# lxtGH/Video-K-Net

Hardware: AMD Instinct MI355X
Metric: frames/sec (S=3, N=100, 1024x2048) (higher is better)
Workload: dtype f32; 1 GPU; cfg2 video_knet_s3_r50: VideoKernelIterHead S=3, N=100 proposals + 17 stuff = 117 kernels, C=256, 1024x2048 frame -> 128x256 stride-8 features, ffn tracking link, x4 bilinear upsample of the final logits; streams_per_gpu=1, parallelism=frame-sharded dp1, x_storage=fp32

## Files before the change

include/vkn.h:

```cpp
#ifndef VKN_H
#define VKN_H
#include <stddef.h>
#include <stdint.h>

#ifdef __cplusplus
extern "C" {
#endif

#define VKN_VERSION 0x000600

#define VKN_OK 0
#define VKN_E_ARG (-1)
#define VKN_E_SHAPE (-2)
#define VKN_E_WORKSPACE (-3)
#define VKN_E_LAUNCH (-4)
#define VKN_E_ALIGN (-5)
#define VKN_E_RANGE (-6)

#define VKN_STATUS_RANGE 1u

#define VKN_FLAG_REF_KERNELS 1u
#define VKN_FLAG_EXACT_GEMM 2u
#define VKN_FLAG_LOGITS_HANDOFF 4u
#define VKN_FLAG_BITS_HANDOFF 16u
#define VKN_X_F32 0
#define VKN_X_F16 1
#define VKN_X_BF16 2
#define VKN_FLAG_X_F16 64u
#define VKN_FLAG_X_BF16 128u
#define VKN_FLAG_CHAIN_LAUNCHES 256u
#define VKN_FLAG_CHAIN_PERSISTENT 512u
#define VKN_FLAG_JOIN_EARLY 32768u
#define VKN_FLAG_LINK_RESERVE 262144u
#define VKN_FLAG_LINK_NO_RESERVE 524288u
#define VKN_FLAG_SCALED_F16 16384u
#define VKN_FLAG_CHAIN_BF16X3 65536u
#define VKN_FLAG_CHAIN_KSPLIT 8192u
#define VKN_FLAG_SERIAL_LINK 32u
#define VKN_FLAG_CLIP_LINK 8u

#define VKN_FLAG_INIT_SEPARATE 131072u
#define VKN_FLAG_PHASE_A 1024u
#define VKN_FLAG_PHASE_B 2048u
#define VKN_FLAG_PHASE_C 4096u
#define VKN_FLAG_PHASE_MASK (VKN_FLAG_PHASE_A | VKN_FLAG_PHASE_B | VKN_FLAG_PHASE_C)

#define VKN_MAX_FCS 4

typedef struct VknDims {
    int B;
    int N;
    int C;
    int H, W;
    int heads;
    int ff;
    int ncls;
    int n_cls_fcs, n_mask_fcs;
    float thr_logit;
    float ln_eps;
} VknDims;

typedef struct VknStageWeights {
    const float *ft_w, *ft_b, *ft_wT;
    const float *dyn_w, *dyn_b;
    const float *inp_w, *inp_b;
    const float *ig_w, *ig_b, *ug_w, *ug_b;
    const float *norm_in_w, *norm_in_b;
    const float *norm_out_w, *norm_out_b;
    const float *inorm_in_w, *inorm_in_b;
// ... 346 lines not shown
```

video-k-net_amd/csrc/vkn_api.hip:

```cpp
#include "../../include/vkn.h"
#include "../../include/vkn_decode.h"
#include "vkn_common.h"
#include "vkn_launch.h"

namespace {

struct Carver {
    char* base;
    size_t off;
    template <class T>
    T* take(size_t n) {
        off = (off + 255) & ~(size_t)255;
        T* p = base ? reinterpret_cast<T*>(base + off) : nullptr;
        off += n * sizeof(T);
        return p;
    }
};

inline bool aligned16(const void* p) { return (reinterpret_cast<uintptr_t>(p) & 15) == 0; }
inline int npt_of(int N) { return (N + 31) / 32 * 32; }

struct StageWs {
    float *part, *cntp, *xraw, *cnt, *xfeat, *params, *inputf, *ig, *ug, *f, *obj1, *qkv, *ao, *obj2, *h, *partial, *t1, *t2,
        *maskfeat, *kb, *kern32, *lq, *lkv, *lobj, *lupd, *lf;
// ... 401 lines not shown
        const long long q = grid * 3 / 4;
        return (int)(q > full ? full : (q < d->B ? d->B : q));
    }
    if (mode != 1 || !persistent_chain || d->B < VKN_LINK_RESERVE_MIN_FRAMES || xdt_of(flags) != 0) return 0;
    return grid == VKN_DECODE_CUS ? full : 0;
}

inline int persistent_min_row_tiles(const PrepW& pw, unsigned flags) {
    return (!(flags & VKN_FLAG_CHAIN_BF16X3) && pw.h2_scale && pw.h2[VKN_H2_DYNFT]) ? 22 : 64;
}
inline unsigned pw_off(const VknStageWeights* w, const void* p) {
    return (unsigned)(static_cast<const char*>(p) - static_cast<const char*>(w->prepared));
}
inline bool chain_weights_ok(const PrepW& pw, bool have_cls) {
    return pw.dynft && pw.dyn && pw.dec && pw.inp && pw.ig && pw.ug && pw.fc && pw.attn_in && pw.attn_out && pw.ffn1 && pw.ffn2 &&
           pw.cls_fc[0] && pw.mask_fc[0] && (!have_cls || pw.fc_cls);
}
inline bool chain_stage_ok(const VknDims* d, const VknStageWeights* w, const PrepW& pw, bool have_cls) {
    return chain_shape_ok(d) && w->prepared && w->prepared_bytes < (1ull << 31) && chain_weights_ok(pw, have_cls) && w->ffn1_w &&
           w->cls_ln_w[0] && w->mask_ln_w[0];
}
bool chain_fast_ok(const VknDims* d, const VknStageWeights* w, const PrepW& pw, unsigned flags, bool have_cls) {
    if (flags & (VKN_FLAG_CHAIN_LAUNCHES | VKN_FLAG_EXACT_GEMM)) return false;
    if (vkn_dbg_env("VKN_CHAIN_LAUNCHES", 0)) return false;
    if (!(flags & VKN_FLAG_CHAIN_PERSISTENT) && !vkn_dbg_env("VKN_CHAIN_PERSISTENT", 0) &&
        (d->B * d->N + 31) / 32 < persistent_min_row_tiles(pw, flags))
        return false;
    return pw.chain_consts && chain_stage_ok(d, w, pw, have_cls);
}
inline bool chain_h2(const PrepW& pw, unsigned flags, bool have_cls) {
    return !(flags & VKN_FLAG_CHAIN_BF16X3) && pw.h2_scale && pw.h2[VKN_H2_DYNFT] && pw.h2[VKN_H2_DEC] && (!have_cls || pw.h2[VKN_H2_FCCLS]);
}

int run_chain_fast(const VknDims* d, const VknStageWeights* w, const PrepW& pw, const float* a0, bool a0_raw, const float* cnt,
                   const float* obj_in, float* obj_out, float* cls_logits, bool cls_sigmoid, float* kern32_out, const StageWs& s,
                   hipStream_t st, bool h2 = false) {
    const int M = d->B * d->N, C = d->C;
    VknChainA a{};
    a.a0 = a0; a.obj_in = obj_in; a.rowscale = a0_raw ? cnt : nullptr;
    a.wbase = w->prepared; a.wbytes = w->prepared_bytes;
    if (h2) {
        a.off_dyn = pw_off(w, pw.h2[a0_raw ? VKN_H2_DYNFT : VKN_H2_DYN]);
        a.off_inp = pw_off(w, pw.h2[VKN_H2_INP]); a.off_ig = pw_off(w, pw.h2[VKN_H2_IG]); a.off_ug = pw_off(w, pw.h2[VKN_H2_UG]);
        a.off_fc = pw_off(w, pw.h2[VKN_H2_FC]); a.off_in = pw_off(w, pw.h2[VKN_H2_IN]);
    } else {
        a.off_dyn = pw_off(w, a0_raw ? pw.dynft : pw.dyn);
        a.off_inp = pw_off(w, pw.inp); a.off_ig = pw_off(w, pw.ig); a.off_ug = pw_off(w, pw.ug); a.off_fc = pw_off(w, pw.fc);
        a.off_in = pw_off(w, pw.attn_in);
    }
    a.consts = pw.chain_consts;
    a.eps = d->ln_eps; a.M = M; a.obj1 = s.obj1; a.qkv = s.qkv; a.status = s.status;
    VKN_TRY(h2 ? vkn_launch_chain_a_h2(a, st) : vkn_launch_chain_a(a, st));
    VKN_TRY(vkn_launch_attn(s.qkv, 3 * C, s.qkv + C, s.qkv + 2 * C, 3 * C, s.ao, C, d->B, d->N, d->N, d->heads, C / d->heads, st));
    VknChainC c{};
    c.ao = s.ao; c.obj1 = s.obj1; c.wbase = w->prepared; c.wbytes = w->prepared_bytes;
    if (h2) {
        c.off_out = pw_off(w, pw.h2[VKN_H2_OUT]); c.off_ffn1 = pw_off(w, pw.h2[VKN_H2_FFN1]); c.off_ffn2 = pw_off(w, pw.h2[VKN_H2_FFN2]);
        c.off_clsfc = pw_off(w, pw.h2[VKN_H2_CLSFC]); c.off_maskfc = pw_off(w, pw.h2[VKN_H2_MASKFC]);
        c.off_fccls = pw.h2[VKN_H2_FCCLS] ? pw_off(w, pw.h2[VKN_H2_FCCLS]) : 0u; c.off_dec = pw_off(w, pw.h2[VKN_H2_DEC]);
    } else {
        c.off_out = pw_off(w, pw.attn_out); c.off_ffn1 = pw_off(w, pw.ffn1); c.off_ffn2 = pw_off(w, pw.ffn2);
        c.off_clsfc = pw_off(w, pw.cls_fc[0]); c.off_maskfc = pw_off(w, pw.mask_fc[0]);
        c.off_fccls = pw.fc_cls ? pw_off(w, pw.fc_cls) : 0u; c.off_dec = pw_off(w, pw.dec);
    }
    c.consts = pw.chain_consts; c.kb0 = pw.kb0;
    c.ff = d->ff; c.ncls = d->ncls; c.cls_sigmoid = cls_sigmoid ? 1 : 0; c.eps = d->ln_eps; c.M = M;
    c.obj_out = obj_out; c.cls_out = cls_logits; c.kb_out = s.kb;
    if (kern32_out) c.kern_out = kern32_out;
    else { c.plane_hi = s.kfh; c.plane_lo = s.kfl; }
    c.rows_per_frame = d->N; c.NPT = npt_of(d->N); c.status = s.status;
    return h2 ? vkn_launch_chain_c_h2(c, st) : vkn_launch_chain_c(c, st);
}

#define VKN_KS_MAX_ROW_TILES 16
inline bool ks_width_ok(const VknDims* d) {
    return chain_width_ok(d) && (d->ff % 512 == 0 || d->ff <= 1024);
}
bool chain_ks_ok(const VknDims* d, const VknStageWeights* w, const PrepW& pw, unsigned flags, bool have_cls) {
    if (flags & (VKN_FLAG_CHAIN_LAUNCHES | VKN_FLAG_CHAIN_PERSISTENT | VKN_FLAG_EXACT_GEMM)) return false;
    if (vkn_dbg_env("VKN_CHAIN_LAUNCHES", 0) || vkn_dbg_env("VKN_CHAIN_PERSISTENT", 0) || !vkn_dbg_env("VKN_CHAIN_KSPLIT", 1)) return false;
    if (!(flags & VKN_FLAG_CHAIN_KSPLIT) && (d->B * d->N + 31) / 32 > VKN_KS_MAX_ROW_TILES) return false;
    if (!ks_width_ok(d) || !chain_stage_ok(d, w, pw, have_cls)) return false;
    const void* v16[] = {w->inorm_in_w, w->inorm_in_b, w->norm_in_w, w->norm_in_b, w->norm_out_w, w->norm_out_b, w->inorm_out_w, w->inorm_out_b,
                         w->fc_norm_w, w->fc_norm_b, w->attn_norm_w, w->attn_norm_b, w->ffn_norm_w, w->ffn_norm_b, w->ffn2_b,
                         w->cls_ln_w[0], w->cls_ln_b[0], w->mask_ln_w[0], w->mask_ln_b[0], pw.dvec};
    for (const void* p : v16)
        if (!p || !aligned16(p)) return false;
    return true;
}

VknKsProb ks_prob(const float* a, int lda, const void* W, int Nout, int KT, float eps) {
    VknKsProb p{};
    p.pro.a[0] = a; p.pro.lda[0] = lda; p.pro.nsum = 1; p.pro.eps = eps;
    p.Wsplit = W; p.Nout = Nout; p.KT = KT;
    return p;
}

int run_chain_ks(const VknDims* d, const VknStageWeights* w, const PrepW& pw, const float* a0, bool a0_raw, const float* cnt,
                 const float* obj_in, float* obj_out, float* cls_logits, bool cls_sigmoid, float* kern32_out, const StageWs& s,
                 hipStream_t st, hipEvent_t obj_ready) {
    const int M = d->B * d->N, C = d->C, FF = d->ff;
    const float eps = d->ln_eps;
    VknKsProb pr[2];
// ... 147 lines not shown
                           will_fast ? w->prepared_bytes : 0));

    float* xfeat = c.x_feat_out ? c.x_feat_out : s.xfeat;
    VknEpi e = mk_epi(d);
    if (given_xfeat) {
        xfeat = const_cast<float*>(c.xfeat_in);
    } else if (has_ft) {
        if (!comp || c.x_feat_out || need_xfeat) {
            e.bias = w->ft_b; e.rowscale = s.cnt; e.out = xfeat; e.ldo = C;
            VKN_TRY(vkn_launch_gemm(s.xraw, nullptr, C, w->ft_w, pw.ft, M, C, C, 1, nullptr, e, st));
        }
    } else {
        if (hipMemcpyAsync(xfeat, s.xraw, (size_t)M * C * sizeof(float), hipMemcpyDeviceToDevice, st) != hipSuccess)
            return VKN_E_LAUNCH;
    }

    const float* obj_in = c.obj_in;
    if (pre_link) {
        PrepW pl;
        VKN_TRY(carve_pw(d, c.link_pre, flags, &pl));
        VKN_TRY(run_link(d, c.link_pre, pl, obj_in, c.prev_pre, s.lobj, s, st, c.link_pre->dyn_w ? xfeat : nullptr, flags));
        obj_in = s.lobj;
    }

    const float* kb = has_ft ? s.kb : nullptr;
    float* const kern32 = ref_decode ? (chain_only ? c.kern_out : s.kern32) : nullptr;
    const bool link = c.prev_obj && c.track_out;
    if (fast) {
        const bool raw = !given_xfeat;
        if (fewrow) {
            VKN_TRY(run_chain_ks(d, w, pw, raw ? s.xraw : xfeat, raw, s.cnt, obj_in, c.obj_out, cls_logits, c.cls_sigmoid, kern32, s, st, c.obj_ready));
        } else {
            VKN_TRY(run_chain_fast(d, w, pw, raw ? s.xraw : xfeat, raw, s.cnt, obj_in, c.obj_out, cls_logits, c.cls_sigmoid, kern32, s, st,
                                   chain_h2(pw, flags, have_cls)));
            if (c.obj_ready && hipEventRecord(c.obj_ready, st) != hipSuccess) return VKN_E_LAUNCH;
        }
        VKN_TRY(emit_masks(d, c, s, ref_decode, s.kern32, kb, touch_nx, touch_nx_bytes, flags, st, !fewrow));
        if (link) VKN_TRY(run_track_link(d, s, st, c.obj_out, c.prev_obj, c.track_out, w, c.link_track, c.track_src, xfeat, flags));
        return VKN_OK;
    }

    VKN_TRY(run_updator(d, w, pw, xfeat, (comp && !given_xfeat) ? s.xraw : nullptr, s.cnt, obj_in, s.obj1, s, st));

    VKN_TRY(run_attention(d, s, s.obj1, s.obj1, d->heads, w->attn_in_w, pw.attn_in, nullptr, w->attn_in_b, w->attn_out_w,
                          pw.attn_out, w->attn_out_b, w->attn_norm_w, w->attn_norm_b, s.obj2, st));
    if (w->ffn1_w) {
        VKN_TRY(run_ffn(d, s, s.obj2, w->ffn1_w, pw.ffn1, w->ffn1_b, w->ffn2_w, pw.ffn2, w->ffn2_b, w->ffn_norm_w,
                        w->ffn_norm_b, c.obj_out, st));
    } else {
        if (hipMemcpyAsync(c.obj_out, s.obj2, (size_t)M * C * sizeof(float), hipMemcpyDeviceToDevice, st) != hipSuccess)
            return VKN_E_LAUNCH;
    }
    const float* obj3 = c.obj_out;

    const bool fork_late = vkn_dbg_env("VKN_LINK_FORK_LATE", 0) != 0;
    if (c.obj_ready && !fork_late && hipEventRecord(c.obj_ready, st) != hipSuccess) return VKN_E_LAUNCH;

    const float* tc = obj3;
    const float* tm = obj3;
    const int nl = d->n_cls_fcs > d->n_mask_fcs ? d->n_cls_fcs : d->n_mask_fcs;
    VknGemmProb pr[2];
    for (int i = 0; i < nl; ++i) {
        int np = 0;
        if (i < d->n_cls_fcs) {
            float* dst = (i & 1) ? s.t2 : s.t1;
            e = mk_epi(d); e.ln_w = w->cls_ln_w[i]; e.ln_b = w->cls_ln_b[i]; e.act = 1; e.out = dst; e.ldo = C;
            pr[np++] = VknGemmProb{tc, nullptr, nullptr, nullptr, C, w->cls_fc_w[i], pw.cls_fc[i], C, e};
// ... 871 lines not shown
```

video-k-net_amd/csrc/vkn_chain.hip:

```cpp
#include "vkn_common.h"
#include "vkn_launch.h"

#ifdef CH_H2
typedef _Float16 ch_e;
#define CH_NPL 2
#define CH_WTILE 32768u
#define k_chain_a k_chain_a_h2
#define k_chain_c k_chain_c_h2
#define ChainAArgs ChainAArgsH2
#define ChainCArgs ChainCArgsH2
#define vkn_launch_chain_a vkn_launch_chain_a_h2
#define vkn_launch_chain_c vkn_launch_chain_c_h2
#else
typedef __bf16 ch_e;
#define CH_NPL 3
#define CH_WTILE 49152u
#endif
typedef ch_e ch_ex8 __attribute__((ext_vector_type(8)));
typedef ch_e ch_ex4 __attribute__((ext_vector_type(4)));
typedef unsigned int cu32x4 __attribute__((ext_vector_type(4)));

#define CH_THREADS 512
#define CH_ROWS 32
#define CH_C 256
#define CH_IMG (CH_NPL * CH_ROWS * CH_C)
#define CH_PLANE (CH_ROWS * CH_C)
#define CH_SBUF (2 * 16 * 32)

#define CH_BAR() asm volatile("s_waitcnt lgkmcnt(0)\n\ts_barrier" ::: "memory")

namespace {

__device__ __forceinline__ void ch_split(float v, ch_e (&p)[CH_NPL]) {
    float r = v;
#pragma unroll
    for (int i = 0; i < CH_NPL; ++i) {
        p[i] = (ch_e)r;
        if (i + 1 < CH_NPL) r -= (float)p[i];
    }
}
__device__ __forceinline__ void ch_split4(const float (&v)[4], ch_ex4 (&o)[CH_NPL]) {
// ... 530 lines not shown
    CC_B2 = 768, CC_FN_W = 1024, CC_FN_B = 1280,
    CC_CLN_W = 1536, CC_CLN_B = 1792,
    CC_MLN_W = 2048, CC_MLN_B = 2304,
    CC_DVEC = 2560,
    CC_CLS_B = 2816,
    CC_DEC_B = 3072,
    CC_B1 = 3328,
    CC_SC = 3328 + 2048,
    CC_TOTAL = 3328 + 2048 + 8
};

struct ChainCArgs {
    const float* ao;
    const float* obj1;
    const void* wbase;
    unsigned wbytes;
    unsigned off_out, off_ffn1, off_ffn2, off_clsfc, off_maskfc, off_fccls, off_dec;
    int nchunks;
    int has_cls;
    int cls_sigmoid;
    int ncls;
    float eps;
    int M;
    const float* kb0;
    float* obj_out;
    float* cls_out;
    float* kb_out;
    _Float16* plane_hi;
    _Float16* plane_lo;
    float* kern_out;
    int rows_per_frame, NPT;
    const float* consts;
    int* status;
};

template <int ABL>
__global__ __launch_bounds__(CH_THREADS) void k_chain_c(const ChainCArgs A) {
    extern __shared__ __attribute__((aligned(16))) char smem_cc[];
    ch_e* IMG0 = reinterpret_cast<ch_e*>(smem_cc);
    ch_e* HID = IMG0 + CH_IMG;
    float* S = reinterpret_cast<float*>(HID + CH_IMG);
    float* CST = S + 2 * CH_SBUF;
#ifdef CH_H2
    float* RS = CST + CC_TOTAL;
#endif

    const int tid = threadIdx.x;
    ChLane L_ = ch_lane(tid);
    L_.status = A.status;
    const ChLane L = L_;
    const int m0 = blockIdx.x * CH_ROWS, M = A.M;
    const int row = m0 + L.li;
    const bool row_ok = row < M;
    const int rowc = min(row, M - 1);
    const __amdgpu_buffer_rsrc_t wrs = __builtin_amdgcn_make_buffer_rsrc(const_cast<void*>(A.wbase), 0, (int)A.wbytes, 0x00020000);

    constexpr int RING = CH_RING_OF(ABL);
    ChRing<RING> R;
    {
        const ChNext first{A.off_out, 0u, 1};
#pragma unroll
        for (int j = 0; j < RING - 1; ++j) ch_wload<RING, CH_AUX_OF(ABL), CH_NP_OF(ABL)>(R, j, wrs, L, first.off(j));
        if (CH_NOLOAD(ABL)) ch_wload<RING>(R, RING - 1, wrs, L, A.off_out);
    }
    ch_stage_consts<CC_TOTAL>(CST, A.consts, tid);
#ifdef CH_H2
    ch_img_load(IMG0, A.ao, CH_C, m0, M, tid, RS);
#else
    ch_img_load(IMG0, A.ao, CH_C, m0, M, tid);
#endif
    float obj[1][16];
    {
        const float* s = A.obj1 + (size_t)rowc * CH_C + L.wave * 32 + 4 * L.g;
#pragma unroll
        for (int q = 0; q < 4; ++q) {
            const f32x4 t = *reinterpret_cast<const f32x4*>(s + 8 * q);
#pragma unroll
            for (int e = 0; e < 4; ++e) obj[0][4 * q + e] = t[e];
        }
    }
    CH_BAR();

    int sb = 0;
    f32x16 acc1[1];
    ch_zero(acc1[0]);
    ch_gemm<1, true, ABL>(acc1, IMG0, IMG0, A.off_out, 0u, ChNext{A.off_ffn1, 0u, 1}, R, wrs, L);
    CH_UNSCALE(acc1[0], CST[CC_SC + 0] * RS[L.li]);
    {
        float b[16];
        ch_cols(CST + CC_OUT_B, L, b);
#pragma unroll
        for (int r = 0; r < 16; ++r) obj[0][r] = acc1[0][r] + b[r] + obj[0][r];
        const float* const lw[1] = {CST + CC_AN_W};
        const float* const lb[1] = {CST + CC_AN_B};
        ch_layernorm<1>(obj, lw, lb, A.eps, S, sb, L);
        ch_img_write(IMG0, obj[0], L);
        CH_BAR();
    }
    f32x16 acc2[1];
    ch_zero(acc2[0]);
#pragma unroll 1
    for (int c = 0; c < A.nchunks; ++c) {
        ch_zero(acc1[0]);
        ch_gemm<1, true, ABL>(acc1, IMG0, IMG0, A.off_ffn1 + (unsigned)c * 8u * CH_WTILE, 0u,
                         ChNext{A.off_ffn2 + (unsigned)c * 8u * CH_WTILE, 0u, 1}, R, wrs, L);
        CH_UNSCALE(acc1[0], CST[CC_SC + 1]);
        float h[16], b[16];
        ch_cols(CST + CC_B1 + 256 * c, L, b);
#pragma unroll
        for (int r = 0; r < 16; ++r) h[r] = fmaxf(acc1[0][r] + b[r], 0.f);
        CH_BAR();
        ch_img_write(HID, h, L);
        CH_BAR();
        const bool lastc = (c + 1 == A.nchunks);
        const ChNext nx = lastc ? ChNext{A.off_clsfc, A.off_maskfc, 2} : ChNext{A.off_ffn1 + (unsigned)(c + 1) * 8u * CH_WTILE, 0u, 1};
        ch_gemm<1, true, ABL>(acc2, HID, HID, A.off_ffn2 + (unsigned)c * 8u * CH_WTILE, 0u, nx, R, wrs, L);
    }
    CH_UNSCALE(acc2[0], CST[CC_SC + 2]);
    {
        float b[16];
        ch_cols(CST + CC_B2, L, b);
#pragma unroll
        for (int r = 0; r < 16; ++r) obj[0][r] = obj[0][r] + acc2[0][r] + b[r];
        const float* const lw[1] = {CST + CC_FN_W};
        const float* const lb[1] = {CST + CC_FN_B};
        ch_layernorm<1>(obj, lw, lb, A.eps, S, sb, L);
        ch_store_rows(A.obj_out, CH_C, 0, row, row_ok, obj[0], L);
        ch_img_write(IMG0, obj[0], L);
        CH_BAR();
    }
    f32x16 acc[2];
    ch_zero(acc[0]);
    ch_zero(acc[1]);
    const ChNext nfin = A.has_cls ? ChNext{A.off_fccls, A.off_dec, 2} : ChNext{A.off_dec, 0u, 1};
    ch_gemm<2, true, ABL>(acc, IMG0, IMG0, A.off_clsfc, A.off_maskfc, nfin, R, wrs, L);
    CH_UNSCALE(acc[0], CST[CC_SC + 3]);
    CH_UNSCALE(acc[1], CST[CC_SC + 4]);
    {
        float t[2][16];
#pragma unroll
        for (int r = 0; r < 16; ++r) {
            t[0][r] = acc[0][r];
            t[1][r] = acc[1][r];
        }
        const float* const lw[2] = {CST + CC_CLN_W, CST + CC_MLN_W};
        const float* const lb[2] = {CST + CC_CLN_B, CST + CC_MLN_B};
        ch_layernorm<2>(t, lw, lb, A.eps, S, sb, L);
        float dv[16], kd[1];
        ch_cols(CST + CC_DVEC, L, dv);
// ... 29 lines not shown
    } else {
        f32x16 accd[1];
        ch_zero(accd[0]);
        ch_gemm<1, true, ABL>(accd, HID, HID, A.off_dec, 0u, ChNext{0u, 0u, 0}, R, wrs, L);
        acc[1] = accd[0];
    }
    CH_UNSCALE(acc[1], CST[CC_SC + 6]);
    {
        float k[16], b[16];
        ch_cols(CST + CC_DEC_B, L, b);
#pragma unroll
        for (int r = 0; r < 16; ++r) k[r] = acc[1][r] + b[r];
        if (A.plane_hi) {
            if (row_ok) {
                const int fb = row / A.rows_per_frame, n = row - fb * A.rows_per_frame;
                const size_t base = ((size_t)fb * A.NPT + n) * CH_C + L.wave * 32 + 4 * L.g;
#pragma unroll
                for (int q = 0; q < 4; ++q) {
                    half4 h, l;
#pragma unroll
                    for (int e = 0; e < 4; ++e) {
                        _Float16 hh, ll;
                        vkn_split_f16(k[4 * q + e], hh, ll);
                        h[e] = hh;
                        l[e] = ll;
                    }
                    *reinterpret_cast<half4*>(A.plane_hi + base + 8 * q) = h;
                    *reinterpret_cast<half4*>(A.plane_lo + base + 8 * q) = l;
                }
            }
        } else {
            ch_store_rows(A.kern_out, CH_C, 0, row, row_ok, k, L);
        }
    }
}

#ifndef CH_H2
template <int ABL, int KC>
__global__ __launch_bounds__(CH_THREADS) void k_gemm_t3(const VknGemmProb p0, const VknGemmProb p1, int nprob, int M) {
    extern __shared__ __attribute__((aligned(16))) char smem_t3[];
    ch_e* IMG = reinterpret_cast<ch_e*>(smem_t3);
    float* S = reinterpret_cast<float*>(IMG + KC * CH_IMG);
    const bool second = (nprob > 1) && (blockIdx.z == 1);
    const VknGemmProb& P = second ? p1 : p0;
    const VknEpi& E = P.epi;
    const int Nout = P.Nout;
    const int m0 = blockIdx.y * CH_ROWS, n0 = blockIdx.x * 256;
    if (n0 >= Nout) return;

    const int tid = threadIdx.x;
    const ChLane L = ch_lane(tid);
    const int ntiles = (Nout + 255) / 256;
    const __amdgpu_buffer_rsrc_t wrs = __builtin_amdgcn_make_buffer_rsrc(const_cast<void*>(P.Wsplit), 0, (int)((unsigned)ntiles * (8u * KC) * CH_WTILE), 0x00020000);
    const unsigned wbase = (unsigned)blockIdx.x * (8u * KC) * CH_WTILE;
    constexpr int RING = CH_RING_OF(ABL);
    ChRing<RING> R;
#pragma unroll
    for (int j = 0; j < RING - 1; ++j) ch_wload<RING, CH_AUX_OF(ABL)>(R, j, wrs, L, wbase + (unsigned)j * CH_WTILE);

#pragma unroll
    for (int kc = 0; kc < KC; ++kc) {
        const int row = tid >> 4, c4 = (tid & 15) << 2;
        const size_t ro = (size_t)min(m0 + row, M - 1) * P.lda + c4 + 256 * kc;
        f32x4 t[4];
#pragma unroll
        for (int j = 0; j < 4; ++j) t[j] = *reinterpret_cast<const f32x4*>(P.A + ro + 64 * j);
// ... 294 lines not shown
        case 2: CHA_LAUNCH(2); break;
        case 3: CHA_LAUNCH(3); break;
        case 4: CHA_LAUNCH(4); break;
        case 5: CHA_LAUNCH(5); break;
        case 6: CHA_LAUNCH(6); break;
        case 7: CHA_LAUNCH(7); break;
        case 8: CHA_LAUNCH(8); break;
        case 9: CHA_LAUNCH(9); break;
        case 10: CHA_LAUNCH(10); break;
        case 11: CHA_LAUNCH(11); break;
        default: CHA_LAUNCH(0); break;
    }
#else
    CHA_LAUNCH(0);
#endif
#undef CHA_LAUNCH
    VKN_CHECK_LAUNCH();
    return VKN_OK;
}

int vkn_launch_chain_c(const VknChainC& p, hipStream_t stream) {
    if (!p.ao || !p.obj1 || !p.wbase || !p.obj_out || !p.consts || p.M <= 0 || p.wbytes >= (1ull << 31)) return VKN_E_ARG;
    if (p.ff <= 0 || p.ff % 256 != 0 || p.ff > 2048 || p.ncls > 256) return VKN_E_SHAPE;
    if (!p.plane_hi == !p.kern_out || (p.plane_hi && !p.plane_lo)) return VKN_E_ARG;
    ChainCArgs A{};
    A.ao = p.ao; A.obj1 = p.obj1; A.wbase = p.wbase; A.wbytes = (unsigned)p.wbytes;
    A.off_out = p.off_out; A.off_ffn1 = p.off_ffn1; A.off_ffn2 = p.off_ffn2; A.off_clsfc = p.off_clsfc; A.off_maskfc = p.off_maskfc;
    A.off_fccls = p.off_fccls; A.off_dec = p.off_dec;
    A.nchunks = p.ff / 256; A.has_cls = (p.cls_out != nullptr) ? 1 : 0; A.cls_sigmoid = p.cls_sigmoid; A.ncls = p.ncls;
    A.eps = p.eps; A.M = p.M; A.kb0 = p.kb0; A.obj_out = p.obj_out; A.cls_out = p.cls_out; A.kb_out = p.kb_out;
    A.plane_hi = p.plane_hi; A.plane_lo = p.plane_lo; A.kern_out = p.kern_out; A.rows_per_frame = p.rows_per_frame; A.NPT = p.NPT;
    A.consts = p.consts + 2 * CA_TOTAL;
    A.status = p.status;
#ifdef CH_H2
    const size_t lds = (size_t)2 * CH_IMG * sizeof(ch_e) + (size_t)(2 * CH_SBUF + CC_TOTAL + 32) * sizeof(float);
#else
    const size_t lds = (size_t)2 * CH_IMG * sizeof(ch_e) + (size_t)(2 * CH_SBUF + CC_TOTAL) * sizeof(float);
#endif
#define CHC_LAUNCH(ABLV)                                                                                            \
    do {                                                                                                            \
        VKN_ALLOW_FULL_LDS(k_chain_c<ABLV>);                                                                        \
        hipLaunchKernelGGL(k_chain_c<ABLV>, dim3((p.M + CH_ROWS - 1) / CH_ROWS), dim3(CH_THREADS), lds, stream, A); \
    } while (0)
#ifdef VKN_DEBUG
    switch (vkn_dbg_env("VKN_CHAIN_ABL", 0)) {
        case 1: CHC_LAUNCH(1); break;
        case 2: CHC_LAUNCH(2); break;
        case 3: CHC_LAUNCH(3); break;
        case 4: CHC_LAUNCH(4); break;
        case 5: CHC_LAUNCH(5); break;
        case 6: CHC_LAUNCH(6); break;
        case 7: CHC_LAUNCH(7); break;
        case 8: CHC_LAUNCH(8); break;
        case 9: CHC_LAUNCH(9); break;
        case 10: CHC_LAUNCH(10); break;
        case 11: CHC_LAUNCH(11); break;
        default: CHC_LAUNCH(0); break;
    }
#else
    CHC_LAUNCH(0);
#endif
#undef CHC_LAUNCH
    VKN_CHECK_LAUNCH();
    return VKN_OK;
}
```

video-k-net_amd/csrc/vkn_launch.h:

```cpp
#pragma once
#include <hip/hip_runtime.h>
#include <stddef.h>

struct VknEpi {
    const float* bias;
    const float* rowscale;
    const float* bias2;
    const float* resid;
    int ldr;
    const float* ln_w;
    const float* ln_b;
    int ln_from_col;
    float eps;
    int act;
    float* out;
    int ldo;
    const float* dot_vec;
    const float* dot_bias;
    float* dot_out;
    _Float16* plane_hi;
    _Float16* plane_lo;
    int rows_per_frame;
    int NPT;
};
// ... 112 lines not shown
int vkn_chain_pack_consts(const VknChainConsts& c, float* out, hipStream_t stream);
struct VknChainA {
    const float* a0;
    const float* obj_in;
    const float* rowscale;
    const void* wbase;
    size_t wbytes;
    unsigned off_dyn, off_inp, off_ig, off_ug, off_fc, off_in;
    const float* consts;
    float eps;
    int M;
    float* obj1;
    float* qkv;
    int* status;
};
struct VknChainC {
    const float* ao;
    const float* obj1;
    const void* wbase;
    size_t wbytes;
    unsigned off_out, off_ffn1, off_ffn2, off_clsfc, off_maskfc, off_fccls, off_dec;
    const float* consts;
    const float* kb0;
    int ff, ncls, cls_sigmoid;
    float eps;
    int M;
    float* obj_out;
    float* cls_out;
    float* kb_out;
    _Float16 *plane_hi, *plane_lo;
    float* kern_out;
    int rows_per_frame, NPT;
    int* status;
};
int vkn_launch_gemm_t3(const VknGemmProb* probs, int nprob, int M, int K, hipStream_t stream);
int vkn_launch_chain_a(const VknChainA& p, hipStream_t stream);
int vkn_launch_chain_c(const VknChainC& p, hipStream_t stream);
int vkn_launch_chain_a_h2(const VknChainA& p, hipStream_t stream);
int vkn_launch_chain_c_h2(const VknChainC& p, hipStream_t stream);
size_t vkn_split_h2_bytes(int Nout, int K);
int vkn_launch_split_h2(const float* W, void* images, int Nout, int K, const float* scale, hipStream_t stream);

struct VknKsPro {
    const float* a[4];
    int lda[4];
    int nsum;
    long long sum_stride;
    const float* pbias;
    const float* presid;
    int ldr;
    const float* ln_w[4];
    const float* ln_b[4];
    float eps;
    int act;
    float* side_out;
    int ld_side;
    const float* dot_vec;
    const float* dot_bias;
    float* dot_out;
};
struct VknKsEpi {
    const float* bias;
    const float* rowscale;
    const float* bias2;
    const float* resid;
    int ldr;
// ... 17 lines not shown
```

video-k-net_amd/ops.py:

```python
import ctypes
import struct
import threading

import torch

from . import _lib
from ._lib import VknDims, VknStageWeights, check

_H = _lib.CONSTS
FLAG_REF_KERNELS = _H['VKN_FLAG_REF_KERNELS']
FLAG_EXACT_GEMM = _H['VKN_FLAG_EXACT_GEMM']
FLAG_LOGITS_HANDOFF = _H['VKN_FLAG_LOGITS_HANDOFF']
FLAG_BITS_HANDOFF = _H['VKN_FLAG_BITS_HANDOFF']
FLAG_CHAIN_LAUNCHES = _H['VKN_FLAG_CHAIN_LAUNCHES']
FLAG_CHAIN_PERSISTENT = _H['VKN_FLAG_CHAIN_PERSISTENT']
FLAG_JOIN_EARLY = _H['VKN_FLAG_JOIN_EARLY']
FLAG_LINK_RESERVE = _H['VKN_FLAG_LINK_RESERVE']
FLAG_LINK_NO_RESERVE = _H['VKN_FLAG_LINK_NO_RESERVE']
FLAG_SCALED_F16 = _H['VKN_FLAG_SCALED_F16']
FLAG_CHAIN_BF16X3 = _H['VKN_FLAG_CHAIN_BF16X3']
FLAG_INIT_SEPARATE = _H['VKN_FLAG_INIT_SEPARATE']
FLAG_CHAIN_KSPLIT = _H['VKN_FLAG_CHAIN_KSPLIT']
FLAG_SERIAL_LINK = _H['VKN_FLAG_SERIAL_LINK']

_tls = threading.local()


def _ptr(t):
    return ctypes.c_void_p(t.data_ptr()) if t is not None else ctypes.c_void_p(0)


def _stream():
    return ctypes.c_void_p(torch.cuda.current_stream().cuda_stream)


def _req(t, name):
    if not torch.is_tensor(t) or not t.is_cuda:
        raise _lib.VknLibraryError(f'{name}: expected a CUDA/HIP tensor — the MI355X path has no CPU fallback')
    if t.dtype != torch.float32:
        raise TypeError(f'{name}: expected float32, got {t.dtype}')
    t = t.contiguous()
    if t.data_ptr() % 16:
        t = t.clone(memory_format=torch.contiguous_format)
    return t


_X_DTYPES = {torch.float32: _H['VKN_X_F32'], torch.float16: _H['VKN_X_F16'], torch.bfloat16: _H['VKN_X_BF16']}
FLAG_X_F16, FLAG_X_BF16 = _H['VKN_FLAG_X_F16'], _H['VKN_FLAG_X_BF16']


def _req_x(t, name='x'):
    if not torch.is_tensor(t) or not t.is_cuda:
        raise _lib.VknLibraryError(f'{name}: expected a CUDA/HIP tensor — the MI355X path has no CPU fallback')
# ... 1259 lines not shown
```

Measured before the change: 9915 frames/s.

## Split chain C kernel across FFN hidden chunks into partial and reduce kernels

```diff
diff --git a/include/vkn.h b/include/vkn.h
--- a/include/vkn.h
+++ b/include/vkn.h
@@ -35,6 +35,7 @@
 #define VKN_FLAG_LINK_NO_RESERVE 524288u
 #define VKN_FLAG_SCALED_F16 16384u
 #define VKN_FLAG_CHAIN_BF16X3 65536u
+#define VKN_FLAG_CHAIN_WHOLE_C 1048576u
 #define VKN_FLAG_CHAIN_KSPLIT 8192u
 #define VKN_FLAG_SERIAL_LINK 32u
 #define VKN_FLAG_CLIP_LINK 8u
diff --git a/video-k-net_amd/csrc/vkn_api.hip b/video-k-net_amd/csrc/vkn_api.hip
--- a/video-k-net_amd/csrc/vkn_api.hip
+++ b/video-k-net_amd/csrc/vkn_api.hip
@@ -457,9 +457,17 @@
     return !(flags & VKN_FLAG_CHAIN_BF16X3) && pw.h2_scale && pw.h2[VKN_H2_DYNFT] && pw.h2[VKN_H2_DEC] && (!have_cls || pw.h2[VKN_H2_FCCLS]);
 }
 
+int chain_c_hsplit(int M, int FF, unsigned flags) {
+    if (flags & VKN_FLAG_CHAIN_WHOLE_C) return 1;
+    const int chunks = FF / 256, rt = (M + 31) / 32;
+    int hs = 1;
+    while (chunks % (hs * 2) == 0 && rt * hs * 2 <= VKN_DECODE_CUS) hs *= 2;
+    return hs;
+}
+
 int run_chain_fast(const VknDims* d, const VknStageWeights* w, const PrepW& pw, const float* a0, bool a0_raw, const float* cnt,
                    const float* obj_in, float* obj_out, float* cls_logits, bool cls_sigmoid, float* kern32_out, const StageWs& s,
-                   hipStream_t st, bool h2 = false) {
+                   hipStream_t st, bool h2 = false, int c_hsplit = 1) {
     const int M = d->B * d->N, C = d->C;
     VknChainA a{};
     a.a0 = a0; a.obj_in = obj_in; a.rowscale = a0_raw ? cnt : nullptr;
@@ -494,6 +502,7 @@
     if (kern32_out) c.kern_out = kern32_out;
     else { c.plane_hi = s.kfh; c.plane_lo = s.kfl; }
     c.rows_per_frame = d->N; c.NPT = npt_of(d->N); c.status = s.status;
+    c.hsplit = c_hsplit; c.obj2 = s.obj2; c.partial = s.partial;
     return h2 ? vkn_launch_chain_c_h2(c, st) : vkn_launch_chain_c(c, st);
 }
 
@@ -707,7 +716,7 @@
             VKN_TRY(run_chain_ks(d, w, pw, raw ? s.xraw : xfeat, raw, s.cnt, obj_in, c.obj_out, cls_logits, c.cls_sigmoid, kern32, s, st, c.obj_ready));
         } else {
             VKN_TRY(run_chain_fast(d, w, pw, raw ? s.xraw : xfeat, raw, s.cnt, obj_in, c.obj_out, cls_logits, c.cls_sigmoid, kern32, s, st,
-                                   chain_h2(pw, flags, have_cls)));
+                                   chain_h2(pw, flags, have_cls), chain_c_hsplit(M, d->ff, flags)));
             if (c.obj_ready && hipEventRecord(c.obj_ready, st) != hipSuccess) return VKN_E_LAUNCH;
         }
         VKN_TRY(emit_masks(d, c, s, ref_decode, s.kern32, kb, touch_nx, touch_nx_bytes, flags, st, !fewrow));
diff --git a/video-k-net_amd/csrc/vkn_chain.hip b/video-k-net_amd/csrc/vkn_chain.hip
--- a/video-k-net_amd/csrc/vkn_chain.hip
+++ b/video-k-net_amd/csrc/vkn_chain.hip
@@ -7,6 +7,8 @@
 #define CH_WTILE 32768u
 #define k_chain_a k_chain_a_h2
 #define k_chain_c k_chain_c_h2
+#define k_chain_c1 k_chain_c1_h2
+#define k_chain_c2 k_chain_c2_h2
 #define ChainAArgs ChainAArgsH2
 #define ChainCArgs ChainCArgsH2
 #define vkn_launch_chain_a vkn_launch_chain_a_h2
@@ -603,7 +605,71 @@
     int rows_per_frame, NPT;
     const float* consts;
     int* status;
+    float* obj2;
+    float* part;
+    int hs;
 };
+
+template <int ABL>
+__device__ __forceinline__ void ch_c_front(const ChainCArgs& A, ch_e* IMG0, float* S, float* CST, float* RS, int& sb, float (&obj)[1][16],
+                                           ChRing<CH_RING_OF(ABL)>& R, const __amdgpu_buffer_rsrc_t wrs, const ChLane& L, int tid, int m0,
+                                           int rowc, const ChNext nx) {
+    constexpr int RING = CH_RING_OF(ABL);
+    {
+        const ChNext first{A.off_out, 0u, 1};
+#pragma unroll
+        for (int j = 0; j < RING - 1; ++j) ch_wload<RING, CH_AUX_OF(ABL), CH_NP_OF(ABL)>(R, j, wrs, L, first.off(j));
+        if (CH_NOLOAD(ABL)) ch_wload<RING>(R, RING - 1, wrs, L, A.off_out);
+    }
+    ch_stage_consts<CC_TOTAL>(CST, A.consts, tid);
+#ifdef CH_H2
+    ch_img_load(IMG0, A.ao, CH_C, m0, A.M, tid, RS);
+#else
+    ch_img_load(IMG0, A.ao, CH_C, m0, A.M, tid);
+#endif
+    {
+        const float* s = A.obj1 + (size_t)rowc * CH_C + L.wave * 32 + 4 * L.g;
+#pragma unroll
+        for (int q = 0; q < 4; ++q) {
+            const f32x4 t = *reinterpret_cast<const f32x4*>(s + 8 * q);
+#pragma unroll
+            for (int e = 0; e < 4; ++e) obj[0][4 * q + e] = t[e];
+        }
+    }
+    CH_BAR();
+
+    f32x16 acc1[1];
+    ch_zero(acc1[0]);
+    ch_gemm<1, true, ABL>(acc1, IMG0, IMG0, A.off_out, 0u, nx, R, wrs, L);
+    CH_UNSCALE(acc1[0], CST[CC_SC + 0] * RS[L.li]);
+    float b[16];
+    ch_cols(CST + CC_OUT_B, L, b);
+#pragma unroll
+    for (int r = 0; r < 16; ++r) obj[0][r] = acc1[0][r] + b[r] + obj[0][r];
+    const float* const lw[1] = {CST + CC_AN_W};
+    const float* const lb[1] = {CST + CC_AN_B};
+    ch_layernorm<1>(obj, lw, lb, A.eps, S, sb, L);
+    ch_img_write(IMG0, obj[0], L);
+    CH_BAR();
+}
+
+template <int ABL>
+__device__ __forceinline__ void ch_ffn_chunk(const ChainCArgs& A, int c, f32x16 (&acc2)[1], const ch_e* IMG0, ch_e* HID, const float* CST,
+                                             ChRing<CH_RING_OF(ABL)>& R, const __amdgpu_buffer_rsrc_t wrs, const ChLane& L, const ChNext nx) {
+    f32x16 acc1[1];
+    ch_zero(acc1[0]);
+    ch_gemm<1, true, ABL>(acc1, IMG0, IMG0, A.off_ffn1 + (unsigned)c * 8u * CH_WTILE, 0u,
+                     ChNext{A.off_ffn2 + (unsigned)c * 8u * CH_WTILE, 0u, 1}, R, wrs, L);
+    CH_UNSCALE(acc1[0], CST[CC_SC + 1]);
+    float h[16], b[16];
+    ch_cols(CST + CC_B1 + 256 * c, L, b);
+#pragma unroll
+    for (int r = 0; r < 16; ++r) h[r] = fmaxf(acc1[0][r] + b[r], 0.f);
+    CH_BAR();
+    ch_img_write(HID, h, L);
+    CH_BAR();
+    ch_gemm<1, true, ABL>(acc2, HID, HID, A.off_ffn2 + (unsigned)c * 8u * CH_WTILE, 0u, nx, R, wrs, L);
+}
 
 template <int ABL>
 __global__ __launch_bounds__(CH_THREADS) void k_chain_c(const ChainCArgs A) {
@@ -614,6 +680,8 @@
     float* CST = S + 2 * CH_SBUF;
 #ifdef CH_H2
     float* RS = CST + CC_TOTAL;
+#else
+    float* RS = nullptr;
 #endif
 
     const int tid = threadIdx.x;
@@ -626,66 +694,17 @@
     const int rowc = min(row, M - 1);
     const __amdgpu_buffer_rsrc_t wrs = __builtin_amdgcn_make_buffer_rsrc(const_cast<void*>(A.wbase), 0, (int)A.wbytes, 0x00020000);
 
-    constexpr int RING = CH_RING_OF(ABL);
-    ChRing<RING> R;
-    {
-        const ChNext first{A.off_out, 0u, 1};
-#pragma unroll
-        for (int j = 0; j < RING - 1; ++j) ch_wload<RING, CH_AUX_OF(ABL), CH_NP_OF(ABL)>(R, j, wrs, L, first.off(j));
-        if (CH_NOLOAD(ABL)) ch_wload<RING>(R, RING - 1, wrs, L, A.off_out);
-    }
-    ch_stage_consts<CC_TOTAL>(CST, A.consts, tid);
-#ifdef CH_H2
-    ch_img_load(IMG0, A.ao, CH_C, m0, M, tid, RS);
-#else
-    ch_img_load(IMG0, A.ao, CH_C, m0, M, tid);
-#endif
+    ChRing<CH_RING_OF(ABL)> R;
+    int sb = 0;
     float obj[1][16];
-    {
-        const float* s = A.obj1 + (size_t)rowc * CH_C + L.wave * 32 + 4 * L.g;
-#pragma unroll
-        for (int q = 0; q < 4; ++q) {
-            const f32x4 t = *reinterpret_cast<const f32x4*>(s + 8 * q);
-#pragma unroll
-            for (int e = 0; e < 4; ++e) obj[0][4 * q + e] = t[e];
-        }
-    }
-    CH_BAR();
-
-    int sb = 0;
-    f32x16 acc1[1];
-    ch_zero(acc1[0]);
-    ch_gemm<1, true, ABL>(acc1, IMG0, IMG0, A.off_out, 0u, ChNext{A.off_ffn1, 0u, 1}, R, wrs, L);
-    CH_UNSCALE(acc1[0], CST[CC_SC + 0] * RS[L.li]);
-    {
-        float b[16];
-        ch_cols(CST + CC_OUT_B, L, b);
-#pragma unroll
-        for (int r = 0; r < 16; ++r) obj[0][r] = acc1[0][r] + b[r] + obj[0][r];
-        const float* const lw[1] = {CST + CC_AN_W};
-        const float* const lb[1] = {CST + CC_AN_B};
-        ch_layernorm<1>(obj, lw, lb, A.eps, S, sb, L);
-        ch_img_write(IMG0, obj[0], L);
-        CH_BAR();
-    }
+    ch_c_front<ABL>(A, IMG0, S, CST, RS, sb, obj, R, wrs, L, tid, m0, rowc, ChNext{A.off_ffn1, 0u, 1});
     f32x16 acc2[1];
     ch_zero(acc2[0]);
 #pragma unroll 1
     for (int c = 0; c < A.nchunks; ++c) {
-        ch_zero(acc1[0]);
-        ch_gemm<1, true, ABL>(acc1, IMG0, IMG0, A.off_ffn1 + (unsigned)c * 8u * CH_WTILE, 0u,
-                         ChNext{A.off_ffn2 + (unsigned)c * 8u * CH_WTILE, 0u, 1}, R, wrs, L);
-        CH_UNSCALE(acc1[0], CST[CC_SC + 1]);
-        float h[16], b[16];
-        ch_cols(CST + CC_B1 + 256 * c, L, b);
-#pragma unroll
-        for (int r = 0; r < 16; ++r) h[r] = fmaxf(acc1[0][r] + b[r], 0.f);
-        CH_BAR();
-        ch_img_write(HID, h, L);
-        CH_BAR();
         const bool lastc = (c + 1 == A.nchunks);
         const ChNext nx = lastc ? ChNext{A.off_clsfc, A.off_maskfc, 2} : ChNext{A.off_ffn1 + (unsigned)(c + 1) * 8u * CH_WTILE, 0u, 1};
-        ch_gemm<1, true, ABL>(acc2, HID, HID, A.off_ffn2 + (unsigned)c * 8u * CH_WTILE, 0u, nx, R, wrs, L);
+        ch_ffn_chunk<ABL>(A, c, acc2, IMG0, HID, CST, R, wrs, L, nx);
     }
     CH_UNSCALE(acc2[0], CST[CC_SC + 2]);
     {
@@ -781,6 +800,195 @@
         } else {
             ch_store_rows(A.kern_out, CH_C, 0, row, row_ok, k, L);
         }
+    }
+}
+
+template <int ABL>
+__global__ __launch_bounds__(CH_THREADS) void k_chain_c1(const ChainCArgs A) {
+    extern __shared__ __attribute__((aligned(16))) char smem_c1[];
+    ch_e* IMG0 = reinterpret_cast<ch_e*>(smem_c1);
+    ch_e* HID = IMG0 + CH_IMG;
+    float* S = reinterpret_cast<float*>(HID + CH_IMG);
+    float* CST = S + 2 * CH_SBUF;
+#ifdef CH_H2
+    float* RS = CST + CC_TOTAL;
+#else
+    float* RS = nullptr;
+#endif
+
+    const int tid = threadIdx.x;
+    ChLane L_ = ch_lane(tid);
+    L_.status = A.status;
+    const ChLane L = L_;
+    const int m0 = blockIdx.x * CH_ROWS, M = A.M;
+    const int row = m0 + L.li;
+    const bool row_ok = row < M;
+    const int rowc = min(row, M - 1);
+    const int grp = blockIdx.y, cpg = A.nchunks / A.hs, cbeg = grp * cpg, cend = cbeg + cpg;
+    const __amdgpu_buffer_rsrc_t wrs = __builtin_amdgcn_make_buffer_rsrc(const_cast<void*>(A.wbase), 0, (int)A.wbytes, 0x00020000);
+
+    ChRing<CH_RING_OF(ABL)> R;
+    int sb = 0;
+    float obj[1][16];
+    ch_c_front<ABL>(A, IMG0, S, CST, RS, sb, obj, R, wrs, L, tid, m0, rowc, ChNext{A.off_ffn1 + (unsigned)cbeg * 8u * CH_WTILE, 0u, 1});
+    if (grp == 0) ch_store_rows(A.obj2, CH_C, 0, row, row_ok, obj[0], L);
+    f32x16 acc2[1];
+    ch_zero(acc2[0]);
+#pragma unroll 1
+    for (int c = cbeg; c < cend; ++c) {
+        const ChNext nx = (c + 1 == cend) ? ChNext{0u, 0u, 0} : ChNext{A.off_ffn1 + (unsigned)(c + 1) * 8u * CH_WTILE, 0u, 1};
+        ch_ffn_chunk<ABL>(A, c, acc2, IMG0, HID, CST, R, wrs, L, nx);
+    }
+    CH_UNSCALE(acc2[0], CST[CC_SC + 2]);
+    {
+        float v[16];
+#pragma unroll
+        for (int r = 0; r < 16; ++r) v[r] = acc2[0][r];
+        ch_store_rows(A.part + (size_t)grp * M * CH_C, CH_C, 0, row, row_ok, v, L);
+    }
+}
+
+template <int ABL>
+__global__ __launch_bounds__(CH_THREADS) void k_chain_c2(const ChainCArgs A) {
+    extern __shared__ __attribute__((aligned(16))) char smem_c2[];
+    ch_e* IMG0 = reinterpret_cast<ch_e*>(smem_c2);
+    float* S = reinterpret_cast<float*>(IMG0 + CH_IMG);
+    float* CST = S + 2 * CH_SBUF;
+
+    const int tid = threadIdx.x;
+    ChLane L_ = ch_lane(tid);
+    L_.status = A.status;
+    const ChLane L = L_;
+    const int m0 = blockIdx.x * CH_ROWS, M = A.M;
+    const int row = m0 + L.li;
+    const bool row_ok = row < M;
+    const int rowc = min(row, M - 1);
+    const bool is_cls = A.has_cls && blockIdx.y == 0;
+    const unsigned off_fc = is_cls ? A.off_clsfc : A.off_maskfc, off_fin = is_cls ? A.off_fccls : A.off_dec;
+    const __amdgpu_buffer_rsrc_t wrs = __builtin_amdgcn_make_buffer_rsrc(const_cast<void*>(A.wbase), 0, (int)A.wbytes, 0x00020000);
+
+    constexpr int RING = CH_RING_OF(ABL);
+    ChRing<RING> R;
+    {
+        const ChNext first{off_fc, 0u, 1};
+#pragma unroll
+        for (int j = 0; j < RING - 1; ++j) ch_wload<RING, CH_AUX_OF(ABL), CH_NP_OF(ABL)>(R, j, wrs, L, first.off(j));
+        if (CH_NOLOAD(ABL)) ch_wload<RING>(R, RING - 1, wrs, L, off_fc);
+    }
+    ch_stage_consts<CC_TOTAL>(CST, A.consts, tid);
+    float obj[1][16];
+    {
+        const size_t ro = (size_t)rowc * CH_C + L.wave * 32 + 4 * L.g;
+        float p[16];
+#pragma unroll
+        for (int r = 0; r < 16; ++r) p[r] = 0.f;
+#pragma unroll 1
+        for (int g0 = 0; g0 < A.hs; g0 += 4) {
+            f32x4 t[4][4];
+#pragma unroll
+            for (int j = 0; j < 4; ++j) {
+                const float* s = A.part + (size_t)min(g0 + j, A.hs - 1) * M * CH_C + ro;
+#pragma unroll
+                for (int q = 0; q < 4; ++q) t[j][q] = *reinterpret_cast<const f32x4*>(s + 8 * q);
+            }
+#pragma unroll
+            for (int j = 0; j < 4; ++j) {
+                if (g0 + j >= A.hs) break;
+#pragma unroll
+                for (int q = 0; q < 4; ++q)
+#pragma unroll
+                    for (int e = 0; e < 4; ++e) p[4 * q + e] = (g0 + j) ? p[4 * q + e] + t[j][q][e] : t[j][q][e];
+            }
+        }
+#pragma unroll
+        for (int q = 0; q < 4; ++q) {
+            const f32x4 t = *reinterpret_cast<const f32x4*>(A.obj2 + ro + 8 * q);
+#pragma unroll
+            for (int e = 0; e < 4; ++e) obj[0][4 * q + e] = t[e];
+        }
+        CH_BAR();
+        float b[16];
+        ch_cols(CST + CC_B2, L, b);
+#pragma unroll
+        for (int r = 0; r < 16; ++r) obj[0][r] = obj[0][r] + p[r] + b[r];
+    }
+    int sb = 0;
+    {
+        const float* const lw[1] = {CST + CC_FN_W};
+        const float* const lb[1] = {CST + CC_FN_B};
+        ch_layernorm<1>(obj, lw, lb, A.eps, S, sb, L);
+        ch_store_rows(A.obj_out, CH_C, 0, row, row_ok && (is_cls || !A.has_cls), obj[0], L);
+        ch_img_write(IMG0, obj[0], L);
+        CH_BAR();
+    }
+    f32x16 acc[1];
+    ch_zero(acc[0]);
+    ch_gemm<1, true, ABL>(acc, IMG0, IMG0, off_fc, 0u, ChNext{off_fin, 0u, 1}, R, wrs, L);
+    CH_UNSCALE(acc[0], CST[CC_SC + (is_cls ? 3 : 4)]);
+    {
+        float t[1][16];
+#pragma unroll
+        for (int r = 0; r < 16; ++r) t[0][r] = acc[0][r];
+        const float* const lw[1] = {CST + (is_cls ? CC_CLN_W : CC_MLN_W)};
+        const float* const lb[1] = {CST + (is_cls ? CC_CLN_B : CC_MLN_B)};
+        ch_layernorm<1>(t, lw, lb, A.eps, S, sb, L);
+#pragma unroll
+        for (int r = 0; r < 16; ++r) t[0][r] = fmaxf(t[0][r], 0.f);
+        ch_img_write(IMG0, t[0], L);
+        if (is_cls) {
+            CH_BAR();
+        } else {
+            float dv[16], kd[1];
+            ch_cols(CST + CC_DVEC, L, dv);
+            kd[0] = 0.f;
+#pragma unroll
+            for (int r = 0; r < 16; ++r) kd[0] += t[0][r] * dv[r];
+            ch_rowsum<1>(kd, S + sb * CH_SBUF, L);
+            sb ^= 1;
+            if (row_ok && L.wave == 0 && L.g == 0 && A.kb_out) A.kb_out[row] = kd[0] + (A.kb0 ? *A.kb0 : 0.f);
+        }
+    }
+    ch_zero(acc[0]);
+    ch_gemm<1, true, ABL>(acc, IMG0, IMG0, off_fin, 0u, ChNext{0u, 0u, 0}, R, wrs, L);
+    CH_UNSCALE(acc[0], CST[CC_SC + (is_cls ? 5 : 6)]);
+    if (is_cls) {
+        if (L.wave * 32 < A.ncls && row_ok && A.cls_out) {
+            float b[16];
+            ch_cols(CST + CC_CLS_B, L, b);
+#pragma unroll
+            for (int r = 0; r < 16; ++r) {
+                const int col = L.wave * 32 + 8 * (r >> 2) + 4 * L.g + (r & 3);
+                float v = acc[0][r] + b[r];
+                if (A.cls_sigmoid) v = 1.0f / (1.0f + expf(-v));
+                if (col < A.ncls) A.cls_out[(size_t)row * A.ncls + col] = v;
+            }
+        }
+        return;
+    }
+    float k[16], b[16];
+    ch_cols(CST + CC_DEC_B, L, b);
+#pragma unroll
+    for (int r = 0; r < 16; ++r) k[r] = acc[0][r] + b[r];
+    if (A.plane_hi) {
+        if (row_ok) {
+            const int fb = row / A.rows_per_frame, n = row - fb * A.rows_per_frame;
+            const size_t base = ((size_t)fb * A.NPT + n) * CH_C + L.wave * 32 + 4 * L.g;
+#pragma unroll
+            for (int q = 0; q < 4; ++q) {
+                half4 h, l;
+#pragma unroll
+                for (int e = 0; e < 4; ++e) {
+                    _Float16 hh, ll;
+                    vkn_split_f16(k[4 * q + e], hh, ll);
+                    h[e] = hh;
+                    l[e] = ll;
+                }
+                *reinterpret_cast<half4*>(A.plane_hi + base + 8 * q) = h;
+                *reinterpret_cast<half4*>(A.plane_lo + base + 8 * q) = l;
+            }
+        }
+    } else {
+        ch_store_rows(A.kern_out, CH_C, 0, row, row_ok, k, L);
     }
 }
 
@@ -1141,15 +1349,26 @@
     A.plane_hi = p.plane_hi; A.plane_lo = p.plane_lo; A.kern_out = p.kern_out; A.rows_per_frame = p.rows_per_frame; A.NPT = p.NPT;
     A.consts = p.consts + 2 * CA_TOTAL;
     A.status = p.status;
+    A.obj2 = p.obj2; A.part = p.partial; A.hs = p.hsplit > 1 ? p.hsplit : 1;
+    if (A.hs > 1 && (!p.obj2 || !p.partial || A.nchunks % A.hs != 0)) return VKN_E_ARG;
 #ifdef CH_H2
     const size_t lds = (size_t)2 * CH_IMG * sizeof(ch_e) + (size_t)(2 * CH_SBUF + CC_TOTAL + 32) * sizeof(float);
 #else
     const size_t lds = (size_t)2 * CH_IMG * sizeof(ch_e) + (size_t)(2 * CH_SBUF + CC_TOTAL) * sizeof(float);
 #endif
-#define CHC_LAUNCH(ABLV)                                                                                            \
-    do {                                                                                                            \
-        VKN_ALLOW_FULL_LDS(k_chain_c<ABLV>);                                                                        \
-        hipLaunchKernelGGL(k_chain_c<ABLV>, dim3((p.M + CH_ROWS - 1) / CH_ROWS), dim3(CH_THREADS), lds, stream, A); \
+    const size_t lds2 = (size_t)CH_IMG * sizeof(ch_e) + (size_t)(2 * CH_SBUF + CC_TOTAL) * sizeof(float);
+    const dim3 rt((p.M + CH_ROWS - 1) / CH_ROWS);
+#define CHC_LAUNCH(ABLV)                                                                                                   \
+    do {                                                                                                                   \
+        if (A.hs > 1) {                            \
+            VKN_ALLOW_FULL_LDS(k_chain_c1<ABLV>);                                                                          \
+            VKN_ALLOW_FULL_LDS(k_chain_c2<ABLV>);                                                                          \
+            hipLaunchKernelGGL(k_chain_c1<ABLV>, dim3(rt.x, A.hs), dim3(CH_THREADS), lds, stream, A);                      \
+            hipLaunchKernelGGL(k_chain_c2<ABLV>, dim3(rt.x, A.has_cls ? 2 : 1), dim3(CH_THREADS), lds2, stream, A);        \
+        } else {                                                                                                           \
+            VKN_ALLOW_FULL_LDS(k_chain_c<ABLV>);                                                                           \
+            hipLaunchKernelGGL(k_chain_c<ABLV>, rt, dim3(CH_THREADS), lds, stream, A);                                     \
+        }                                                                                                                  \
     } while (0)
 #ifdef VKN_DEBUG
     switch (vkn_dbg_env("VKN_CHAIN_ABL", 0)) {
diff --git a/video-k-net_amd/csrc/vkn_launch.h b/video-k-net_amd/csrc/vkn_launch.h
--- a/video-k-net_amd/csrc/vkn_launch.h
+++ b/video-k-net_amd/csrc/vkn_launch.h
@@ -168,6 +168,9 @@
     float* kern_out;
     int rows_per_frame, NPT;
     int* status;
+    int hsplit;
+    float* obj2;
+    float* partial;
 };
 int vkn_launch_gemm_t3(const VknGemmProb* probs, int nprob, int M, int K, hipStream_t stream);
 int vkn_launch_chain_a(const VknChainA& p, hipStream_t stream);
diff --git a/video-k-net_amd/ops.py b/video-k-net_amd/ops.py
--- a/video-k-net_amd/ops.py
+++ b/video-k-net_amd/ops.py
@@ -19,6 +19,7 @@
 FLAG_LINK_NO_RESERVE = _H['VKN_FLAG_LINK_NO_RESERVE']
 FLAG_SCALED_F16 = _H['VKN_FLAG_SCALED_F16']
 FLAG_CHAIN_BF16X3 = _H['VKN_FLAG_CHAIN_BF16X3']
+FLAG_CHAIN_WHOLE_C = _H['VKN_FLAG_CHAIN_WHOLE_C']
 FLAG_INIT_SEPARATE = _H['VKN_FLAG_INIT_SEPARATE']
 FLAG_CHAIN_KSPLIT = _H['VKN_FLAG_CHAIN_KSPLIT']
 FLAG_SERIAL_LINK = _H['VKN_FLAG_SERIAL_LINK']
```

Result: faster. 10030 frames/s, median of 6 (+1.1%).
